# pierluigiferrari/lane_tracker

Hardware: NVIDIA B200
Metric: frames/sec at 1280x720 (batched streams) (higher is better)
Workload: dtype u8

## Files before the change

### lane_tracker_b200/csrc/lt_morph.cu

```cuda
#include <cstdlib>
#include <cstdio>
#include <algorithm>
#include <functional>
#include <vector>
#include <map>
#include <mutex>
#include <tuple>
#include <cstring>
#include <cuda.h>
#include "lt_common.cuh"
#include "lt_ellipse.cuh"

namespace {

constexpr int TW = 192;
#ifndef LT_MORPH_NPW
#define LT_MORPH_NPW 2
#endif
constexpr int NPW = LT_MORPH_NPW;
#ifndef LT_MORPH_UNROLL4
#define LT_MORPH_UNROLL4 4
#endif
#ifndef LT_MORPH_UNROLL8
#define LT_MORPH_UNROLL8 4
#endif
#ifndef LT_MORPH_T32_FROM_T16
#define LT_MORPH_T32_FROM_T16 0
#endif
constexpr int UNROLL4 = LT_MORPH_UNROLL4, UNROLL8 = LT_MORPH_UNROLL8;
constexpr int NPROD = 32 * NPW;
constexpr int NTHREADS = TW + NPROD;
constexpr int RB = 8, RP = RB / 2;

constexpr int BAR_FULL = 1, BAR_EMPTY = 3, BAR_PROD = 5;

__device__ __forceinline__ void bar_sync(int id, int count) { asm volatile("bar.sync %0, %1;" ::"r"(id), "r"(count) : "memory"); }
__device__ __forceinline__ void bar_arrive(int id, int count) { asm volatile("bar.arrive %0, %1;" ::"r"(id), "r"(count) : "memory"); }

__device__ __forceinline__ void cp_async16(void* smem_dst, const void* gsrc) {
    unsigned sa = (unsigned)__cvta_generic_to_shared(smem_dst);
    asm volatile("cp.async.cg.shared.global [%0], [%1], 16;\n" ::"r"(sa), "l"(gsrc) : "memory");
}
__device__ __forceinline__ void cp_async_commit() { asm volatile("cp.async.commit_group;\n" ::: "memory"); }
__device__ __forceinline__ void cp_async_wait_all() { asm volatile("cp.async.wait_all;\n" ::: "memory"); }

__device__ __forceinline__ void mbar_init(uint64_t* bar, int count) {
    asm volatile("mbarrier.init.shared::cta.b64 [%0], %1;" ::"r"((unsigned)__cvta_generic_to_shared(bar)), "r"(count) : "memory");
}
__device__ __forceinline__ void mbar_expect_tx(uint64_t* bar, unsigned bytes) {
    asm volatile("mbarrier.arrive.expect_tx.shared::cta.b64 _, [%0], %1;" ::"r"((unsigned)__cvta_generic_to_shared(bar)), "r"(bytes) : "memory");
}
__device__ __forceinline__ void mbar_wait(uint64_t* bar, unsigned parity) {
    asm volatile(
        "{\n.reg .pred p;\nWAIT_%=:\n"
        "mbarrier.try_wait.parity.shared::cta.b64 p, [%0], %1;\n"
        "@!p bra WAIT_%=;\n}\n" ::"r"((unsigned)__cvta_generic_to_shared(bar)), "r"(parity) : "memory");
}
__device__ __forceinline__ void tma_load_2d(void* smem_dst, const CUtensorMap* map, int x, int y, uint64_t* bar) {
    asm volatile("cp.async.bulk.tensor.2d.shared::cluster.global.mbarrier::complete_tx::bytes [%0], [%1, {%2, %3}], [%4];"
                 ::"r"((unsigned)__cvta_generic_to_shared(smem_dst)), "l"(map), "r"(x), "r"(y),
                   "r"((unsigned)__cvta_generic_to_shared(bar)) : "memory");
}
__device__ __forceinline__ void fence_proxy_async() { asm volatile("fence.proxy.async.shared::cta;" ::: "memory"); }

template <bool IS_MAX> __device__ __forceinline__ uint32_t op2(uint32_t a, uint32_t b) { return IS_MAX ? __vmaxu2(a, b) : __vminu2(a, b); }
template <bool IS_MAX> __device__ __forceinline__ uint32_t op3(uint32_t a, uint32_t b, uint32_t c) {
    return IS_MAX ? __vimax3_u16x2(a, b, c) : __vimin3_u16x2(a, b, c);
}

template <int K> struct Geo {
    using E = Ellipse<K>;
    static constexpr int R = E::R;
    static constexpr int HA = (R + 3) & ~3;
    static constexpr int TE = TW + 2 * HA;
    static constexpr int TEA = TE + 32;
    static constexpr bool HAS32 = (2 * R + 1) >= 32;
    static constexpr int NCT = HAS32 ? 4 : 3;
    static constexpr int CH = TE / 4;
    static constexpr int TBUF = NCT * RP * TEA;
    static constexpr int TEP = TE + 4;
    static constexpr int PRIV = RP * TEA + 2 * RB * TEP;
    static constexpr int OGW = 2 * RB * TW;
    static constexpr size_t smem(bool tophat) { return (size_t)(2 * TBUF + PRIV + (tophat ? OGW : 0)) * sizeof(uint32_t) + 32; }
    static_assert((2 * TBUF + RP * TEA) % 32 == 0 && (RB * TEP) % 32 == 0 && TE <= 256, "the raw row buffers must be 128-byte aligned for the TMA variant");
    static_assert((2 * TBUF + PRIV) % 32 == 0 && (RB * TW) % 32 == 0, "so must the original-row buffers");
    static_assert(HA >= R && HA <= LT_HALO_X && R + RB <= LT_HALO_Y && TE % 4 == 0, "staging must be 16-byte granular and inside the plane padding");
};

template <int K, bool IS_MAX>
__device__ __forceinline__ void pair_step(const uint32_t (&S)[K], uint32_t (&D)[K], uint32_t& out_a, const uint32_t* __restrict__ T,
                                          int base) {
    using G = Geo<K>;
    using E = Ellipse<K>;
    constexpr int TS = RP * G::TEA;
    auto H = [&](int w, uint32_t& ha, uint32_t& hb) {
        const int len = 2 * w + 1;
        if (w == 0) { const uint32_t t = T[base]; ha = t << 8; hb = t; return; }
        const uint32_t* tab = len >= 32 ? T + 3 * TS : (len >= 16 ? T + 2 * TS : T + TS);
        const int k = len >= 32 ? 32 : (len >= 16 ? 16 : 8);
        const uint32_t l = tab[base - w], r = tab[base + w - k + 1];
        ha = op2<IS_MAX>(l << 8, r << 8);
        hb = op2<IS_MAX>(l, r);
    };
    uint32_t a0, b0, a1, b1;
    H(E::hw(0), a0, b0);
    out_a = op2<IS_MAX>(S[1], a0);
    D[K - 1] = b0;
#pragma unroll
    for (int j = 0; j <= (K - 3) / 2; ++j) {
        if (E::hw(j + 1) != E::hw(j)) H(E::hw(j + 1), a1, b1); else { a1 = a0; b1 = b0; }
        D[j] = op3<IS_MAX>(S[j + 2], a1, b0);
        const int q = K - 2 - j;
        if (q != j) {
            if (q + 2 < K) D[q] = op3<IS_MAX>(S[q + 2], a0, b1);
            else D[q] = op2<IS_MAX>(a0, b1);
        }
        a0 = a1; b0 = b1;
    }
}

struct MorphArgs {
    const uint32_t* src; uint32_t* dst; const uint32_t* orig;
    int bands, band_rows, tiles, n, sms;
    size_t stride;
    const int* list; const int* count;
};

template <int K, bool IS_MAX, bool TOPHAT, int MINB, bool TMA>
__global__ void __launch_bounds__(NTHREADS, MINB)
k_morph(MorphArgs a, LtDims d, const __grid_constant__ CUtensorMap tmap, const __grid_constant__ CUtensorMap omap) {
    using G = Geo<K>;
    using E = Ellipse<K>;
    constexpr int R = G::R, HA = G::HA, TEA = G::TEA;
    constexpr uint32_t PADL = IS_MAX ? 0u : 0xFFFFu, PAD2 = PADL | (PADL << 16);

    int item = blockIdx.x;
    const int slot = item % a.n;
    item /= a.n;
    const int tile = item % a.tiles, band = item / a.tiles;
    if (a.count != nullptr && slot >= *a.count) return;
    const int s = a.list ? a.list[slot] : slot;
    const uint32_t* src = a.src + (size_t)s * a.stride;
    uint32_t* dst = a.dst + (size_t)s * a.stride;
    const int pitch = d.pp;

    extern __shared__ __align__(128) uint32_t smem[];
    uint32_t* const TB = smem;
    uint32_t* const T4 = smem + 2 * G::TBUF;
    uint32_t* const RAW = T4 + RP * TEA;
    uint32_t* const OG = RAW + 2 * RB * G::TEP;
    uint64_t* const mbar = reinterpret_cast<uint64_t*>(smem + 2 * G::TBUF + G::PRIV + (TOPHAT ? G::OGW : 0));

    const int x0 = tile * TW;
    const int yb0 = band * a.band_rows;
    const int yb1 = min(yb0 + a.band_rows, d.bv_h);
    const int r_begin = yb0 - R;
    const int r_end = yb1 + R;
    const int nblk = (r_end - r_begin + RB - 1) / RB;

    const int warp = threadIdx.x >> 5, lane = threadIdx.x & 31;
    const int pfirst = ((blockIdx.x / a.sms) & 1) ? 4 : 6;
    const bool producer = warp >= pfirst && warp < pfirst + NPW;
    const int tid = ((warp >= pfirst + NPW ? warp - NPW : warp) << 5) | lane;

    if (producer) {
        constexpr int TEP = G::TEP;
        const int pt = ((warp - pfirst) << 5) | lane;
        constexpr int TPR = NPROD / RB;
        const int srow = pt / TPR, sc0 = pt % TPR;
        const uint32_t* sp = src + (ptrdiff_t)(r_begin + srow) * pitch + (x0 - HA) + 4 * sc0;
        uint32_t* const sdst = RAW + srow * TEP + 4 * sc0;
        auto stage = [&](int buf) {
            uint32_t* t = sdst + buf * RB * TEP;
#pragma unroll
            for (int c = 0; c < G::CH; c += TPR)
                if (c + sc0 < G::CH) cp_async16(t + 4 * c, sp + 4 * c);
            sp += (ptrdiff_t)RB * pitch;
            cp_async_commit();
        };
        const uint32_t* op = TOPHAT ? a.orig + (size_t)s * a.stride + (ptrdiff_t)(r_begin - R + srow) * pitch + x0 + 4 * sc0 : nullptr;
        uint32_t* const odst = OG + srow * TW + 4 * sc0;
        int oy = r_begin - R + srow;
        auto stage_orig = [&](int buf) {
            if ((unsigned)oy < (unsigned)d.bv_h) {
                uint32_t* t = odst + buf * RB * TW;
#pragma unroll
                for (int c = 0; c < TW / 4; c += TPR)
                    if (c + sc0 < TW / 4) cp_async16(t + 4 * c, op + 4 * c);
            }
            op += (ptrdiff_t)RB * pitch;
            oy += RB;
            cp_async_commit();
        };
        constexpr int RPITCH = TMA ? G::TE : TEP;
        constexpr unsigned BLOCK_BYTES = RB * G::TE * sizeof(uint32_t);
        const int tx = LT_HALO_X + x0 - HA;
        int ty = s * (d.bv_h + 2 * LT_HALO_Y) + LT_HALO_Y + r_begin;
        auto stage_tma = [&](int buf) {
            if (pt == 0) {
                fence_proxy_async();
                mbar_expect_tx(&mbar[buf], BLOCK_BYTES);
                tma_load_2d(RAW + buf * RB * TEP, &tmap, tx, ty, &mbar[buf]);
            }
            ty += RB;
        };
        const int ox = LT_HALO_X + x0;
        int oyt = s * (d.bv_h + 2 * LT_HALO_Y) + LT_HALO_Y + r_begin - R;
        auto stage_orig_tma = [&](int buf) {
            if (pt == 0) {
                fence_proxy_async();
                mbar_expect_tx(&mbar[2 + buf], (unsigned)(RB * TW * sizeof(uint32_t)));
                tma_load_2d(OG + buf * RB * TW, &omap, ox, oyt, &mbar[2 + buf]);
            }
            oyt += RB;
        };
        if (TMA) {
            if (pt == 0) {
                mbar_init(&mbar[0], 1); mbar_init(&mbar[1], 1); mbar_init(&mbar[2], 1); mbar_init(&mbar[3], 1);
                asm volatile("fence.mbarrier_init.release.cluster;" ::: "memory");
            }
            bar_sync(BAR_PROD, NPROD);
            stage_tma(0);
        } else {
            stage(0);
        }
        for (int blk = 0; blk < nblk; ++blk) {
            const int b = blk & 1;
            if (TMA) mbar_wait(&mbar[b], (unsigned)(blk >> 1) & 1u); else cp_async_wait_all();
            bar_sync(BAR_PROD, NPROD);
            if (blk + 1 < nblk) { if (TMA) stage_tma(b ^ 1); else stage(b ^ 1); }
            if (blk >= 2) bar_sync(BAR_EMPTY + b, NTHREADS);
            if (TOPHAT) { if (TMA) stage_orig_tma(b); else stage_orig(b); }
            uint32_t* const Tb = TB + b * G::TBUF;
            const uint32_t* const Rw = RAW + b * RB * TEP;
            constexpr int NTASK = RP * G::CH, NIT = (NTASK + NPROD - 1) / NPROD;
#pragma unroll UNROLL4
            for (int it = 0; it < NIT; ++it) {
                const int q = pt + it * NPROD;
                if (q >= NTASK) break;
                const int pr = q / G::CH, c = (q - pr * G::CH) * 4;
                const uint4* ra = reinterpret_cast<const uint4*>(Rw + (2 * pr) * RPITCH + c);
                const uint4* rb = reinterpret_cast<const uint4*>(Rw + (2 * pr + 1) * RPITCH + c);
                const uint4 a0 = ra[0], a1 = ra[1], b0 = rb[0], b1 = rb[1];
                uint4 t1;
                t1.x = __byte_perm(a0.x, b0.x, 0x6240); t1.y = __byte_perm(a0.y, b0.y, 0x6240);
                t1.z = __byte_perm(a0.z, b0.z, 0x6240); t1.w = __byte_perm(a0.w, b0.w, 0x6240);
                *reinterpret_cast<uint4*>(Tb + pr * TEA + c) = t1;
                auto win4 = [](const uint4& u, const uint4& v, uint32_t (&e)[4]) {
                    const uint32_t m01 = op2<IS_MAX>(u.x, u.y), m23 = op2<IS_MAX>(u.z, u.w), m45 = op2<IS_MAX>(v.x, v.y);
                    e[0] = op2<IS_MAX>(m01, m23);
                    e[1] = op3<IS_MAX>(u.y, m23, v.x);
                    e[2] = op2<IS_MAX>(m23, m45);
                    e[3] = op3<IS_MAX>(u.w, m45, v.z);
                };
                uint32_t ea[4], eb[4];
                win4(a0, a1, ea);
                win4(b0, b1, eb);
                uint4 t4;
                t4.x = __byte_perm(ea[0], eb[0], 0x6240); t4.y = __byte_perm(ea[1], eb[1], 0x6240);
                t4.z = __byte_perm(ea[2], eb[2], 0x6240); t4.w = __byte_perm(ea[3], eb[3], 0x6240);
                *reinterpret_cast<uint4*>(T4 + pr * TEA + c) = t4;
            }
            bar_sync(BAR_PROD, NPROD);
            constexpr bool T32_DIRECT = G::HAS32 && !LT_MORPH_T32_FROM_T16;
#pragma unroll UNROLL8
            for (int it = 0; it < NIT; ++it) {
                const int q = pt + it * NPROD;
                if (q >= NTASK) break;
                const int pr = q / G::CH, c = (q - pr * G::CH) * 4;
                const uint4* t = reinterpret_cast<const uint4*>(T4 + pr * TEA + c);
                uint4 v[T32_DIRECT ? 8 : 4];
#pragma unroll
                for (int k = 0; k < (T32_DIRECT ? 8 : 4); ++k) v[k] = t[k];
                uint32_t o8[4], o16[4], o32[4];
#pragma unroll
                for (int e = 0; e < 4; ++e) {
                    auto w = [&](int k) { const uint4& u = v[k]; return e == 0 ? u.x : (e == 1 ? u.y : (e == 2 ? u.z : u.w)); };
                    const uint32_t a8 = op2<IS_MAX>(w(0) << 8, w(1) << 8), b8 = op2<IS_MAX>(w(0), w(1));
                    const uint32_t a16 = op3<IS_MAX>(a8, w(2) << 8, w(3) << 8), b16 = op3<IS_MAX>(b8, w(2), w(3));
                    o8[e] = __byte_perm(a8, b8, 0x7351);
                    o16[e] = __byte_perm(a16, b16, 0x7351);
                    if (T32_DIRECT) {
                        const uint32_t a32 = op3<IS_MAX>(a16, op2<IS_MAX>(w(4) << 8, w(5) << 8), op2<IS_MAX>(w(6) << 8, w(7) << 8));
                        const uint32_t b32 = op3<IS_MAX>(b16, op2<IS_MAX>(w(4), w(5)), op2<IS_MAX>(w(6), w(7)));
                        o32[e] = __byte_perm(a32, b32, 0x7351);
                    }
                }
                uint32_t* o = Tb + RP * TEA + pr * TEA + c;
                *reinterpret_cast<uint4*>(o) = make_uint4(o8[0], o8[1], o8[2], o8[3]);
                *reinterpret_cast<uint4*>(o + RP * TEA) = make_uint4(o16[0], o16[1], o16[2], o16[3]);
                if (T32_DIRECT) *reinterpret_cast<uint4*>(o + 2 * RP * TEA) = make_uint4(o32[0], o32[1], o32[2], o32[3]);
            }
            if (G::HAS32 && !T32_DIRECT) {
                bar_sync(BAR_PROD, NPROD);
#pragma unroll UNROLL8
                for (int it = 0; it < NIT; ++it) {
                    const int q = pt + it * NPROD;
                    if (q >= NTASK) break;
                    const int pr = q / G::CH, c = (q - pr * G::CH) * 4;
                    const uint32_t* t16 = Tb + 2 * RP * TEA + pr * TEA + c;
                    const uint4 u = *reinterpret_cast<const uint4*>(t16), v = *reinterpret_cast<const uint4*>(t16 + 16);
                    auto m = [](uint32_t x, uint32_t y) {
                        return __byte_perm(op2<IS_MAX>(x << 8, y << 8), op2<IS_MAX>(x, y), 0x7351);
                    };
                    *reinterpret_cast<uint4*>(Tb + 3 * RP * TEA + pr * TEA + c) = make_uint4(m(u.x, v.x), m(u.y, v.y), m(u.z, v.z), m(u.w, v.w));
                }
            }
            if (TOPHAT) { if (TMA) mbar_wait(&mbar[2 + b], (unsigned)(blk >> 1) & 1u); else cp_async_wait_all(); }
            bar_arrive(BAR_FULL + b, NTHREADS);
        }
        return;
    }

    const int gx = x0 + tid;
    const bool col_ok = gx < d.p2;
    const bool hi_real = gx + d.p2 < d.bv_w;
    const uint32_t sel_out = hi_real ? 0x4341u : 0x4441u;
    const uint32_t lane_mask = hi_real ? 0xFFFFFFFFu : 0x0000FFFFu;
    int hoff = 0;
    uint32_t hsel = 0;
    if (!TOPHAT && col_ok) {
        if (gx >= d.p2 - LT_HALO_X) { hoff = -d.p2; hsel = 0x1044u; }
        else if (gx < LT_HALO_X) { hoff = d.p2; hsel = 0x4432u; }
    }
    uint32_t* dp = dst + (ptrdiff_t)(r_begin - R) * pitch + gx;

    uint32_t A[K], B[K];
#pragma unroll
    for (int j = 0; j < K; ++j) A[j] = PAD2;

    int ya = r_begin - R;
    for (int blk = 0; blk < nblk; ++blk) {
        const int b = blk & 1;
        bar_sync(BAR_FULL + b, NTHREADS);
        const uint32_t* const Tb = TB + b * G::TBUF;
        if (col_ok) {
            int base = tid + HA;
            const uint32_t* ogp = OG + b * RB * TW + tid;
#pragma unroll
            for (int m = 0; m < RP; m += 2) {
#pragma unroll
                for (int h = 0; h < 2; ++h, base += TEA, ya += 2, dp += 2 * (ptrdiff_t)pitch, ogp += 2 * TW) {
                    uint32_t out_a, out_b;
                    if (h == 0) { pair_step<K, IS_MAX>(A, B, out_a, Tb, base); out_b = B[0]; }
                    else { pair_step<K, IS_MAX>(B, A, out_a, Tb, base); out_b = A[0]; }
                    if (ya < yb0 || ya >= yb1) continue;
                    uint32_t va = __byte_perm(out_a, 0, sel_out), vb = __byte_perm(out_b, 0, sel_out);
                    if (TOPHAT) { va = (ogp[0] - va) & lane_mask; vb = (ogp[TW] - vb) & lane_mask; }
                    const bool eb = ya + 1 < yb1;
                    dp[0] = va;
                    if (eb) dp[pitch] = vb;
                    if (!TOPHAT && hsel) {
                        dp[hoff] = __byte_perm(va, 0, hsel);
                        if (eb) dp[hoff + pitch] = __byte_perm(vb, 0, hsel);
                    }
                }
            }
        } else {
            ya += 2 * RP;
        }
        if (blk + 2 < nblk) bar_arrive(BAR_EMPTY + b, NTHREADS);
    }
}

static int plane_tensor_map(lt_handle* h, const uint32_t* plane, int box_w, CUtensorMap* out) {
    typedef CUresult (*EncodeFn)(CUtensorMap*, CUtensorMapDataType, cuuint32_t, void*, const cuuint64_t*, const cuuint64_t*,
                                 const cuuint32_t*, const cuuint32_t*, CUtensorMapInterleave, CUtensorMapSwizzle,
                                 CUtensorMapL2promotion, CUtensorMapFloatOOBfill);
    static EncodeFn encode = nullptr;
    static std::mutex mu;
    static std::map<std::tuple<int, const void*, int, long long, int>, CUtensorMap> cache;
    std::lock_guard<std::mutex> lock(mu);
    if (!encode) {
        void* fn = nullptr;
        cudaDriverEntryPointQueryResult qres;
        if (cudaGetDriverEntryPoint("cuTensorMapEncodeTiled", &fn, cudaEnableDefault, &qres) != cudaSuccess || !fn) {
            lt_set_error("cuTensorMapEncodeTiled is not available");
            return -2;
        }
        encode = (EncodeFn)fn;
    }
    const LtDims& d = h->d;
    const uint32_t* base = plane - ((size_t)LT_HALO_Y * d.pp + LT_HALO_X);
    const long long rows = (long long)h->S * (d.bv_h + 2 * LT_HALO_Y) + 1;
    const auto key = std::make_tuple(h->cfg.device, (const void*)base, d.pp, rows, box_w);
    auto it = cache.find(key);
    if (it == cache.end()) {
        CUtensorMap m;
        const cuuint64_t dims[2] = {(cuuint64_t)d.pp, (cuuint64_t)rows};
        const cuuint64_t strides[1] = {(cuuint64_t)d.pp * sizeof(uint32_t)};
        const cuuint32_t box[2] = {(cuuint32_t)box_w, (cuuint32_t)RB}, estr[2] = {1, 1};
        CUresult r = encode(&m, CU_TENSOR_MAP_DATA_TYPE_UINT32, 2, (void*)base, dims, strides, box, estr, CU_TENSOR_MAP_INTERLEAVE_NONE,
                            CU_TENSOR_MAP_SWIZZLE_NONE, CU_TENSOR_MAP_L2_PROMOTION_L2_128B, CU_TENSOR_MAP_FLOAT_OOB_FILL_NONE);
        if (r != CUDA_SUCCESS) { lt_set_error("cuTensorMapEncodeTiled failed (%d)", (int)r); return -2; }
        it = cache.emplace(key, m).first;
    }
    *out = it->second;
    return 0;
}

template <int K, bool IS_MAX, bool TOPHAT, int MINB>
int launch_occ(lt_handle* h, const uint32_t* src, uint32_t* dst, const uint32_t* orig, int bands, int n, const int* list,
               const int* count, cudaStream_t st) {
    const LtDims& d = h->d;
    MorphArgs a;
    a.src = src; a.dst = dst; a.orig = orig;
    a.band_rows = (lt_div_up(d.bv_h, bands) + 1) & ~1;
    a.bands = lt_div_up(d.bv_h, a.band_rows);
    a.tiles = lt_div_up(d.p2, TW);
    a.n = n; a.stride = h->stream_pad; a.list = list; a.count = count;
    a.sms = h->sm_count > 0 ? h->sm_count : 148;
    static const bool parity = [] { const char* e = getenv("LT_MORPH_PARITY"); return e && e[0] == '1'; }();
    if (!parity) a.sms = 1 << 30;
    static const bool tma = [] { const char* e = getenv("LT_MORPH_TMA"); return !(e && e[0] == '0'); }();
    CUtensorMap tm;
    memset(&tm, 0, sizeof(tm));
    int rc;
    CUtensorMap om = tm;
    if (tma) {
        if ((rc = plane_tensor_map(h, src, Geo<K>::TE, &tm))) return rc;
        if (TOPHAT && (rc = plane_tensor_map(h, orig, TW, &om))) return rc;
        if ((rc = lt_ensure_smem((const void*)k_morph<K, IS_MAX, TOPHAT, MINB, true>, Geo<K>::smem(TOPHAT)))) return rc;
        k_morph<K, IS_MAX, TOPHAT, MINB, true><<<n * a.tiles * a.bands, NTHREADS, Geo<K>::smem(TOPHAT), st>>>(a, d, tm, om);
    } else {
        if ((rc = lt_ensure_smem((const void*)k_morph<K, IS_MAX, TOPHAT, MINB, false>, Geo<K>::smem(TOPHAT)))) return rc;
        k_morph<K, IS_MAX, TOPHAT, MINB, false><<<n * a.tiles * a.bands, NTHREADS, Geo<K>::smem(TOPHAT), st>>>(a, d, tm, om);
    }
    LT_LAUNCH_CHECK();
    return 0;
}

template <int K, bool IS_MAX, bool TOPHAT>
int launch_one(lt_handle* h, const uint32_t* src, uint32_t* dst, const uint32_t* orig, int bands, int n, const int* list,
               const int* count, cudaStream_t st) {
    return launch_occ<K, IS_MAX, TOPHAT, K == 55 ? 2 : 3>(h, src, dst, orig, bands, n, list, count, st);
}

}

int lt_plane_tensor_map(lt_handle* h, const uint32_t* plane, int box_w, CUtensorMap* out) { return plane_tensor_map(h, plane, box_w, out); }

static void choose_bands(lt_handle* h, int n, int tiles, int H, int* b55, int* b29) {
    const int sms = h->sm_count > 0 ? h->sm_count : 148;
    if (h->bands_key[0] == n && h->bands_key[1] == H && h->bands_key[2] == sms) { *b55 = h->bands_val[0]; *b29 = h->bands_val[1]; return; }
    int c55 = 1, c29 = 1;
    bool fixed = false;
    if (const char* ov = getenv("LT_MORPH_BANDS")) {
        if (sscanf(ov, "%d,%d", &c55, &c29) == 2 && c55 >= 1 && c29 >= 1) fixed = true;
        else c55 = c29 = 1;
    }
    if (!fixed) {
        double best = 1e300;
        std::vector<double> freeat;
        for (int a = 1; a <= 16; ++a)
            for (int b = 1; b <= 16; ++b) {
                const int ra = (lt_div_up(H, a) + 1) & ~1, rb = (lt_div_up(H, b) + 1) & ~1;
                const int na = n * tiles * lt_div_up(H, ra), nb = n * tiles * lt_div_up(H, rb);
                const double ta = (ra + 56) * 1.0, tb = (rb + 30) * 0.55;
                const int slots = (7 * sms) / 2;
                freeat.assign(slots, 0.0);
                std::make_heap(freeat.begin(), freeat.end(), std::greater<double>());
                double makespan = 0.0;
                for (int i = 0; i < na + nb; ++i) {
                    std::pop_heap(freeat.begin(), freeat.end(), std::greater<double>());
                    const double t = freeat.back() + (i < na ? ta : tb);
                    freeat.back() = t;
                    std::push_heap(freeat.begin(), freeat.end(), std::greater<double>());
                    if (t > makespan) makespan = t;
                }
                if (makespan < best - 1e-9) { best = makespan; c55 = a; c29 = b; }
            }
    }
    h->bands_key[0] = n; h->bands_key[1] = H; h->bands_key[2] = sms;
    h->bands_val[0] = c55; h->bands_val[1] = c29;
    *b55 = c55; *b29 = c29;
}

int lt_launch_morph_pair(lt_handle* h, bool tophat, int n, const int* list, const int* count, cudaStream_t st) {
    const LtDims& d = h->d;
    int b55, b29, rc;
    choose_bands(h, n, lt_div_up(d.p2, TW), d.bv_h, &b55, &b29);
    cudaStream_t s2 = h->side ? h->side : st;
    if (s2 != st) {
        LT_CUDA(cudaEventRecord(h->ev_fork, st));
        LT_CUDA(cudaStreamWaitEvent(s2, h->ev_fork, 0));
    }
    if (!tophat) {
        if ((rc = launch_one<55, false, false>(h, h->planeB, h->tmpB, nullptr, b55, n, list, count, st))) return rc;
        if ((rc = launch_one<29, false, false>(h, h->planeR, h->tmpR, nullptr, b29, n, list, count, s2))) return rc;
    } else {
        if ((rc = launch_one<55, true, true>(h, h->tmpB, h->topB, h->planeB, b55, n, list, count, st))) return rc;
        if ((rc = launch_one<29, true, true>(h, h->tmpR, h->topR, h->planeR, b29, n, list, count, s2))) return rc;
    }
    if (s2 != st) {
        LT_CUDA(cudaEventRecord(h->ev_join, s2));
        LT_CUDA(cudaStreamWaitEvent(st, h->ev_join, 0));
    }
    return 0;
}
```

Measured before the change: 53410.

## Generalize morph producer/consumer ring to configurable stage depth, drop cp.async path

Replaces the fixed double-buffered transposed-tile ring with an NT-stage ring (2 for erode, 3 for tophat by default) and a separate raw-row TMA ring whose depth shrinks to 2 if shared memory would not fit MINB CTAs. Producers can now run further ahead of the consumer warps, which is meant to hide TMA and barrier latency. The non-TMA cp.async fallback is removed, and optional clock64 probes are added behind a compile flag. The cost is more shared memory per CTA, which could lower occupancy, plus more named barriers.

```diff
diff --git a/lane_tracker_b200/csrc/lt_morph.cu b/lane_tracker_b200/csrc/lt_morph.cu
--- a/lane_tracker_b200/csrc/lt_morph.cu
+++ b/lane_tracker_b200/csrc/lt_morph.cu
@@ -31,18 +31,47 @@
 constexpr int NPROD = 32 * NPW;
 constexpr int NTHREADS = TW + NPROD;
 constexpr int RB = 8, RP = RB / 2;
-
-constexpr int BAR_FULL = 1, BAR_EMPTY = 3, BAR_PROD = 5;
+#ifdef LT_MORPH_STAGES
+#define LT_MORPH_STAGES_ERODE LT_MORPH_STAGES
+#define LT_MORPH_STAGES_TOPHAT LT_MORPH_STAGES
+#endif
+#ifndef LT_MORPH_STAGES_ERODE
+#define LT_MORPH_STAGES_ERODE 2
+#endif
+#ifndef LT_MORPH_STAGES_TOPHAT
+#define LT_MORPH_STAGES_TOPHAT 3
+#endif
 
 __device__ __forceinline__ void bar_sync(int id, int count) { asm volatile("bar.sync %0, %1;" ::"r"(id), "r"(count) : "memory"); }
 __device__ __forceinline__ void bar_arrive(int id, int count) { asm volatile("bar.arrive %0, %1;" ::"r"(id), "r"(count) : "memory"); }
 
-__device__ __forceinline__ void cp_async16(void* smem_dst, const void* gsrc) {
-    unsigned sa = (unsigned)__cvta_generic_to_shared(smem_dst);
-    asm volatile("cp.async.cg.shared.global [%0], [%1], 16;\n" ::"r"(sa), "l"(gsrc) : "memory");
-}
-__device__ __forceinline__ void cp_async_commit() { asm volatile("cp.async.commit_group;\n" ::: "memory"); }
-__device__ __forceinline__ void cp_async_wait_all() { asm volatile("cp.async.wait_all;\n" ::: "memory"); }
+#ifndef LT_MORPH_PROBE
+#define LT_MORPH_PROBE 0
+#endif
+enum { PR_FULL, PR_EMPTY, PR_TMA, PR_TOTAL, PR_N };
+#if LT_MORPH_PROBE
+__device__ unsigned long long g_morph_probe[4][2][4][PR_N];
+#endif
+struct Probe {
+#if LT_MORPH_PROBE
+    long long acc[PR_N], t0;
+    __device__ __forceinline__ void start() { acc[0] = acc[1] = acc[2] = 0; t0 = clock64(); }
+    template <class F> __device__ __forceinline__ void wait(int c, F&& f) {
+        const long long t = clock64();
+        f();
+        acc[c] += clock64() - t;
+    }
+    __device__ __forceinline__ void finish(int kernel, int role, int warp) {
+        acc[PR_TOTAL] = clock64() - t0;
+        if ((threadIdx.x & 31) == 0)
+            for (int c = 0; c < PR_N; ++c) atomicAdd(&g_morph_probe[kernel][role][warp & 3][c], (unsigned long long)acc[c]);
+    }
+#else
+    __device__ __forceinline__ void start() {}
+    template <class F> __device__ __forceinline__ void wait(int, F&& f) { f(); }
+    __device__ __forceinline__ void finish(int, int, int) {}
+#endif
+};
 
 __device__ __forceinline__ void mbar_init(uint64_t* bar, int count) {
     asm volatile("mbarrier.init.shared::cta.b64 [%0], %1;" ::"r"((unsigned)__cvta_generic_to_shared(bar)), "r"(count) : "memory");
@@ -78,13 +107,24 @@
     static constexpr int NCT = HAS32 ? 4 : 3;
     static constexpr int CH = TE / 4;
     static constexpr int TBUF = NCT * RP * TEA;
-    static constexpr int TEP = TE + 4;
-    static constexpr int PRIV = RP * TEA + 2 * RB * TEP;
-    static constexpr int OGW = 2 * RB * TW;
-    static constexpr size_t smem(bool tophat) { return (size_t)(2 * TBUF + PRIV + (tophat ? OGW : 0)) * sizeof(uint32_t) + 32; }
-    static_assert((2 * TBUF + RP * TEA) % 32 == 0 && (RB * TEP) % 32 == 0 && TE <= 256, "the raw row buffers must be 128-byte aligned for the TMA variant");
-    static_assert((2 * TBUF + PRIV) % 32 == 0 && (RB * TW) % 32 == 0, "so must the original-row buffers");
+    static constexpr int RBUF = RB * (TE + 4);
+    static_assert(TBUF % 32 == 0 && (RP * TEA) % 32 == 0 && RBUF % 32 == 0 && TE <= 256, "the raw row buffers must be 128-byte aligned for TMA");
+    static_assert((RB * TW) % 32 == 0, "so must the original-row buffers");
     static_assert(HA >= R && HA <= LT_HALO_X && R + RB <= LT_HALO_Y && TE % 4 == 0, "staging must be 16-byte granular and inside the plane padding");
+};
+
+template <int K, bool TOPHAT, int MINB> struct Ring {
+    using G = Geo<K>;
+    static constexpr int NT = TOPHAT ? LT_MORPH_STAGES_TOPHAT : LT_MORPH_STAGES_ERODE;
+    static constexpr int BAR_FULL = 1, BAR_EMPTY = BAR_FULL + NT, BAR_PROD = BAR_EMPTY + NT;
+    static_assert(NT >= 2 && BAR_PROD < 16, "a CTA has 16 named barriers");
+    static constexpr size_t bytes(int nr) {
+        return (size_t)(NT * G::TBUF + RP * G::TEA + nr * G::RBUF + (TOPHAT ? NT * RB * TW : 0)) * sizeof(uint32_t) + 8 * (nr + NT);
+    }
+    static constexpr size_t SM_BYTES = 228 * 1024, CTA_RESERVED = 1024;
+    static constexpr int NR = MINB * (bytes(NT) + CTA_RESERVED) <= SM_BYTES ? NT : 2;
+    static constexpr size_t SMEM = bytes(NR);
+    static_assert(MINB * (SMEM + CTA_RESERVED) <= SM_BYTES, "MINB CTAs must fit the shared memory of an SM");
 };
 
 template <int K, bool IS_MAX>
@@ -120,19 +160,24 @@
 }
 
 struct MorphArgs {
-    const uint32_t* src; uint32_t* dst; const uint32_t* orig;
+    uint32_t* dst;
     int bands, band_rows, tiles, n, sms;
     size_t stride;
     const int* list; const int* count;
 };
 
-template <int K, bool IS_MAX, bool TOPHAT, int MINB, bool TMA>
+template <int K, bool IS_MAX, bool TOPHAT, int MINB>
 __global__ void __launch_bounds__(NTHREADS, MINB)
 k_morph(MorphArgs a, LtDims d, const __grid_constant__ CUtensorMap tmap, const __grid_constant__ CUtensorMap omap) {
     using G = Geo<K>;
     using E = Ellipse<K>;
-    constexpr int R = G::R, HA = G::HA, TEA = G::TEA;
+    using RG = Ring<K, TOPHAT, MINB>;
+    constexpr int R = G::R, HA = G::HA, TEA = G::TEA, NT = RG::NT, NR = RG::NR;
+    constexpr int BAR_FULL = RG::BAR_FULL, BAR_EMPTY = RG::BAR_EMPTY, BAR_PROD = RG::BAR_PROD;
     constexpr uint32_t PADL = IS_MAX ? 0u : 0xFFFFu, PAD2 = PADL | (PADL << 16);
+    constexpr int PKERNEL = (K == 55 ? 0 : 2) + (TOPHAT ? 1 : 0);
+    Probe probe;
+    probe.start();
 
     int item = blockIdx.x;
     const int slot = item % a.n;
@@ -140,16 +185,15 @@
     const int tile = item % a.tiles, band = item / a.tiles;
     if (a.count != nullptr && slot >= *a.count) return;
     const int s = a.list ? a.list[slot] : slot;
-    const uint32_t* src = a.src + (size_t)s * a.stride;
     uint32_t* dst = a.dst + (size_t)s * a.stride;
     const int pitch = d.pp;
 
     extern __shared__ __align__(128) uint32_t smem[];
     uint32_t* const TB = smem;
-    uint32_t* const T4 = smem + 2 * G::TBUF;
+    uint32_t* const T4 = smem + NT * G::TBUF;
     uint32_t* const RAW = T4 + RP * TEA;
-    uint32_t* const OG = RAW + 2 * RB * G::TEP;
-    uint64_t* const mbar = reinterpret_cast<uint64_t*>(smem + 2 * G::TBUF + G::PRIV + (TOPHAT ? G::OGW : 0));
+    uint32_t* const OG = RAW + NR * G::RBUF;
+    uint64_t* const mbar = reinterpret_cast<uint64_t*>(OG + (TOPHAT ? NT * RB * TW : 0));
 
     const int x0 = tile * TW;
     const int yb0 = band * a.band_rows;
@@ -164,83 +208,54 @@
     const int tid = ((warp >= pfirst + NPW ? warp - NPW : warp) << 5) | lane;
 
     if (producer) {
-        constexpr int TEP = G::TEP;
         const int pt = ((warp - pfirst) << 5) | lane;
-        constexpr int TPR = NPROD / RB;
-        const int srow = pt / TPR, sc0 = pt % TPR;
-        const uint32_t* sp = src + (ptrdiff_t)(r_begin + srow) * pitch + (x0 - HA) + 4 * sc0;
-        uint32_t* const sdst = RAW + srow * TEP + 4 * sc0;
-        auto stage = [&](int buf) {
-            uint32_t* t = sdst + buf * RB * TEP;
-#pragma unroll
-            for (int c = 0; c < G::CH; c += TPR)
-                if (c + sc0 < G::CH) cp_async16(t + 4 * c, sp + 4 * c);
-            sp += (ptrdiff_t)RB * pitch;
-            cp_async_commit();
-        };
-        const uint32_t* op = TOPHAT ? a.orig + (size_t)s * a.stride + (ptrdiff_t)(r_begin - R + srow) * pitch + x0 + 4 * sc0 : nullptr;
-        uint32_t* const odst = OG + srow * TW + 4 * sc0;
-        int oy = r_begin - R + srow;
-        auto stage_orig = [&](int buf) {
-            if ((unsigned)oy < (unsigned)d.bv_h) {
-                uint32_t* t = odst + buf * RB * TW;
-#pragma unroll
-                for (int c = 0; c < TW / 4; c += TPR)
-                    if (c + sc0 < TW / 4) cp_async16(t + 4 * c, op + 4 * c);
-            }
-            op += (ptrdiff_t)RB * pitch;
-            oy += RB;
-            cp_async_commit();
-        };
-        constexpr int RPITCH = TMA ? G::TE : TEP;
         constexpr unsigned BLOCK_BYTES = RB * G::TE * sizeof(uint32_t);
         const int tx = LT_HALO_X + x0 - HA;
         int ty = s * (d.bv_h + 2 * LT_HALO_Y) + LT_HALO_Y + r_begin;
-        auto stage_tma = [&](int buf) {
+        int rq = 0;
+        auto stage = [&]() {
             if (pt == 0) {
                 fence_proxy_async();
-                mbar_expect_tx(&mbar[buf], BLOCK_BYTES);
-                tma_load_2d(RAW + buf * RB * TEP, &tmap, tx, ty, &mbar[buf]);
+                mbar_expect_tx(&mbar[rq], BLOCK_BYTES);
+                tma_load_2d(RAW + rq * G::RBUF, &tmap, tx, ty, &mbar[rq]);
             }
             ty += RB;
+            if (++rq == NR) rq = 0;
         };
         const int ox = LT_HALO_X + x0;
         int oyt = s * (d.bv_h + 2 * LT_HALO_Y) + LT_HALO_Y + r_begin - R;
-        auto stage_orig_tma = [&](int buf) {
+        auto stage_orig = [&](int buf) {
             if (pt == 0) {
                 fence_proxy_async();
-                mbar_expect_tx(&mbar[2 + buf], (unsigned)(RB * TW * sizeof(uint32_t)));
-                tma_load_2d(OG + buf * RB * TW, &omap, ox, oyt, &mbar[2 + buf]);
+                mbar_expect_tx(&mbar[NR + buf], (unsigned)(RB * TW * sizeof(uint32_t)));
+                tma_load_2d(OG + buf * RB * TW, &omap, ox, oyt, &mbar[NR + buf]);
             }
             oyt += RB;
         };
-        if (TMA) {
-            if (pt == 0) {
-                mbar_init(&mbar[0], 1); mbar_init(&mbar[1], 1); mbar_init(&mbar[2], 1); mbar_init(&mbar[3], 1);
-                asm volatile("fence.mbarrier_init.release.cluster;" ::: "memory");
-            }
+        if (pt == 0) {
+            for (int i = 0; i < NR + (TOPHAT ? NT : 0); ++i) mbar_init(&mbar[i], 1);
+            asm volatile("fence.mbarrier_init.release.cluster;" ::: "memory");
+        }
+        bar_sync(BAR_PROD, NPROD);
+        for (int i = 0; i < NR - 1 && i < nblk; ++i) stage();
+        int rbuf = 0, b = 0;
+        unsigned rph = 0, tph = 0;
+        for (int blk = 0; blk < nblk; ++blk) {
+            probe.wait(PR_TMA, [&] { mbar_wait(&mbar[rbuf], rph); });
             bar_sync(BAR_PROD, NPROD);
-            stage_tma(0);
-        } else {
-            stage(0);
-        }
-        for (int blk = 0; blk < nblk; ++blk) {
-            const int b = blk & 1;
-            if (TMA) mbar_wait(&mbar[b], (unsigned)(blk >> 1) & 1u); else cp_async_wait_all();
-            bar_sync(BAR_PROD, NPROD);
-            if (blk + 1 < nblk) { if (TMA) stage_tma(b ^ 1); else stage(b ^ 1); }
-            if (blk >= 2) bar_sync(BAR_EMPTY + b, NTHREADS);
-            if (TOPHAT) { if (TMA) stage_orig_tma(b); else stage_orig(b); }
+            if (blk + NR - 1 < nblk) stage();
+            if (blk >= NT) probe.wait(PR_EMPTY, [&] { bar_sync(BAR_EMPTY + b, NTHREADS); });
+            if (TOPHAT) stage_orig(b);
             uint32_t* const Tb = TB + b * G::TBUF;
-            const uint32_t* const Rw = RAW + b * RB * TEP;
+            const uint32_t* const Rw = RAW + rbuf * G::RBUF;
             constexpr int NTASK = RP * G::CH, NIT = (NTASK + NPROD - 1) / NPROD;
 #pragma unroll UNROLL4
             for (int it = 0; it < NIT; ++it) {
                 const int q = pt + it * NPROD;
                 if (q >= NTASK) break;
                 const int pr = q / G::CH, c = (q - pr * G::CH) * 4;
-                const uint4* ra = reinterpret_cast<const uint4*>(Rw + (2 * pr) * RPITCH + c);
-                const uint4* rb = reinterpret_cast<const uint4*>(Rw + (2 * pr + 1) * RPITCH + c);
+                const uint4* ra = reinterpret_cast<const uint4*>(Rw + (2 * pr) * G::TE + c);
+                const uint4* rb = reinterpret_cast<const uint4*>(Rw + (2 * pr + 1) * G::TE + c);
                 const uint4 a0 = ra[0], a1 = ra[1], b0 = rb[0], b1 = rb[1];
                 uint4 t1;
                 t1.x = __byte_perm(a0.x, b0.x, 0x6240); t1.y = __byte_perm(a0.y, b0.y, 0x6240);
@@ -306,9 +321,12 @@
                     *reinterpret_cast<uint4*>(Tb + 3 * RP * TEA + pr * TEA + c) = make_uint4(m(u.x, v.x), m(u.y, v.y), m(u.z, v.z), m(u.w, v.w));
                 }
             }
-            if (TOPHAT) { if (TMA) mbar_wait(&mbar[2 + b], (unsigned)(blk >> 1) & 1u); else cp_async_wait_all(); }
+            if (TOPHAT) probe.wait(PR_TMA, [&] { mbar_wait(&mbar[NR + b], tph); });
             bar_arrive(BAR_FULL + b, NTHREADS);
+            if (++rbuf == NR) { rbuf = 0; rph ^= 1u; }
+            if (++b == NT) { b = 0; tph ^= 1u; }
         }
+        probe.finish(PKERNEL, 1, warp);
         return;
     }
 
@@ -331,8 +349,8 @@
 
     int ya = r_begin - R;
     for (int blk = 0; blk < nblk; ++blk) {
-        const int b = blk & 1;
-        bar_sync(BAR_FULL + b, NTHREADS);
+        const int b = blk % NT;
+        probe.wait(PR_FULL, [&] { bar_sync(BAR_FULL + b, NTHREADS); });
         const uint32_t* const Tb = TB + b * G::TBUF;
         if (col_ok) {
             int base = tid + HA;
@@ -359,8 +377,9 @@
         } else {
             ya += 2 * RP;
         }
-        if (blk + 2 < nblk) bar_arrive(BAR_EMPTY + b, NTHREADS);
-    }
+        if (blk + NT < nblk) bar_arrive(BAR_EMPTY + b, NTHREADS);
+    }
+    probe.finish(PKERNEL, 0, warp);
 }
 
 static int plane_tensor_map(lt_handle* h, const uint32_t* plane, int box_w, CUtensorMap* out) {
@@ -404,7 +423,7 @@
                const int* count, cudaStream_t st) {
     const LtDims& d = h->d;
     MorphArgs a;
-    a.src = src; a.dst = dst; a.orig = orig;
+    a.dst = dst;
     a.band_rows = (lt_div_up(d.bv_h, bands) + 1) & ~1;
     a.bands = lt_div_up(d.bv_h, a.band_rows);
     a.tiles = lt_div_up(d.p2, TW);
@@ -412,20 +431,15 @@
     a.sms = h->sm_count > 0 ? h->sm_count : 148;
     static const bool parity = [] { const char* e = getenv("LT_MORPH_PARITY"); return e && e[0] == '1'; }();
     if (!parity) a.sms = 1 << 30;
-    static const bool tma = [] { const char* e = getenv("LT_MORPH_TMA"); return !(e && e[0] == '0'); }();
     CUtensorMap tm;
     memset(&tm, 0, sizeof(tm));
     int rc;
     CUtensorMap om = tm;
-    if (tma) {
-        if ((rc = plane_tensor_map(h, src, Geo<K>::TE, &tm))) return rc;
-        if (TOPHAT && (rc = plane_tensor_map(h, orig, TW, &om))) return rc;
-        if ((rc = lt_ensure_smem((const void*)k_morph<K, IS_MAX, TOPHAT, MINB, true>, Geo<K>::smem(TOPHAT)))) return rc;
-        k_morph<K, IS_MAX, TOPHAT, MINB, true><<<n * a.tiles * a.bands, NTHREADS, Geo<K>::smem(TOPHAT), st>>>(a, d, tm, om);
-    } else {
-        if ((rc = lt_ensure_smem((const void*)k_morph<K, IS_MAX, TOPHAT, MINB, false>, Geo<K>::smem(TOPHAT)))) return rc;
-        k_morph<K, IS_MAX, TOPHAT, MINB, false><<<n * a.tiles * a.bands, NTHREADS, Geo<K>::smem(TOPHAT), st>>>(a, d, tm, om);
-    }
+    if ((rc = plane_tensor_map(h, src, Geo<K>::TE, &tm))) return rc;
+    if (TOPHAT && (rc = plane_tensor_map(h, orig, TW, &om))) return rc;
+    constexpr size_t smem = Ring<K, TOPHAT, MINB>::SMEM;
+    if ((rc = lt_ensure_smem((const void*)k_morph<K, IS_MAX, TOPHAT, MINB>, smem))) return rc;
+    k_morph<K, IS_MAX, TOPHAT, MINB><<<n * a.tiles * a.bands, NTHREADS, smem, st>>>(a, d, tm, om);
     LT_LAUNCH_CHECK();
     return 0;
 }
@@ -439,6 +453,17 @@
 }
 
 int lt_plane_tensor_map(lt_handle* h, const uint32_t* plane, int box_w, CUtensorMap* out) { return plane_tensor_map(h, plane, box_w, out); }
+
+#if LT_MORPH_PROBE
+extern "C" int lt_morph_probe_read(unsigned long long* out, int reset) {
+    if (cudaDeviceSynchronize() != cudaSuccess || cudaMemcpyFromSymbol(out, g_morph_probe, sizeof(g_morph_probe)) != cudaSuccess) return -1;
+    if (reset) {
+        static unsigned long long zero[sizeof(g_morph_probe) / sizeof(unsigned long long)];
+        if (cudaMemcpyToSymbol(g_morph_probe, zero, sizeof(g_morph_probe)) != cudaSuccess) return -1;
+    }
+    return (int)(sizeof(g_morph_probe) / sizeof(unsigned long long));
+}
+#endif
 
 static void choose_bands(lt_handle* h, int n, int tiles, int H, int* b55, int* b29) {
     const int sms = h->sm_count > 0 ? h->sm_count : 148;
```

Result: no change. 53890, median of 6 (+0.9%).
